# salesforce/ai-economist

Hardware: AMD Instinct MI355X
Metric: agent-steps/sec, gather-trade-build 25x25 4-agent batched envs (higher is better)
Workload: dtype u8/i32 state + f64 coin/utility (f32 observations); 1 GPU; C2 BASELINE configs[1]: gather-trade-build 25x25, 4 agents + planner, Build+CDA+Gather+PeriodicBracketTax, 4096 replicas/GPU, uniform random policy, planner not counted; envs_per_gpu=4096, global_envs=4096, n_agents=4, kernel_specialisation=compile time, parallelism=single GPU

## Files before the change

### ai-economist_amd/csrc/aie_capi.hip

```cpp
#include <hip/hip_runtime.h>

#include <cstdio>
#include <cstdlib>
#include <cstring>
#include <vector>

#include "aie_kernels.hip"
#include "aie_kernels_ose.hip"
#include "aie_kernels_saez.hip"
#include "aie_kernels_covid.hip"
#include "aie_jit.h"

struct aie_env {
  aie_params P{};
  aie_params* d_params;
  aie_tensor_table tt;
  uint8_t* arena;
  bool owns_arena;
  size_t vmm_total, vmm_piece;
  int device;
  size_t lds;
  int spec;
  int spec_match;
  hipModule_t jit_mod;
  hipFunction_t jit_step, jit_reset;
  std::shared_ptr<aie_jit::Job> jit_job;
  int pinned_generic;
  float* rew_log;
  int32_t rew_log_slots, rew_log_epoch;
  int cv_taps_f32;
  int log_active;
  char err[512];
};

static thread_local char g_create_err[512] = "";
static inline void aie_jit_poll(aie_env* env);
static bool aie_jit_eligible(const aie_env* env);
static int aie_jit_request(aie_env* env);

#define AIE_DEV_API __attribute__((visibility("default")))

#define AIE_HIP_CHECK(env, expr)                                                          \
  do {                                                                                    \
    hipError_t _e = (expr);                                                               \
    if (_e != hipSuccess) {                                                               \
      snprintf((env)->err, sizeof((env)->err), "%s failed: %s", #expr, hipGetErrorString(_e)); \
      return AIE_E_HIP;                                                                   \
    }                                                                                     \
  } while (0)

static uint8_t* aie_arena_alloc_pieces(int device, size_t bytes, size_t piece_mb, size_t* vmm_total, size_t* vmm_piece);
static uint8_t* aie_arena_alloc(int device, size_t bytes, size_t* vmm_total, size_t* vmm_piece) {
  const char* e_min = getenv("AIE_ARENA_VMM_MIN_MB");
  const char* e_piece = getenv("AIE_ARENA_PIECE_MB");
  const size_t min_mb = e_min ? (size_t)atol(e_min) : 1024;
  return aie_arena_alloc_pieces(device, bytes, bytes >= (min_mb << 20) ? (e_piece ? (size_t)atol(e_piece) : 64) : 0, vmm_total, vmm_piece);
}
static uint8_t* aie_arena_alloc_pieces(int device, size_t bytes, size_t piece_mb, size_t* vmm_total, size_t* vmm_piece) {
  *vmm_total = *vmm_piece = 0;
  void* p = nullptr;
  if (piece_mb > 0) {
    hipMemAllocationProp prop = {};
    prop.type = hipMemAllocationTypePinned;
    prop.location.type = hipMemLocationTypeDevice;
    prop.location.id = device;
    size_t gran = 0;
    if (hipMemGetAllocationGranularity(&gran, &prop, hipMemAllocationGranularityMinimum) == hipSuccess && gran > 0) {
      if (gran < ((size_t)2 << 20)) gran = (size_t)2 << 20;
      size_t piece = (piece_mb << 20) / gran * gran;
      if (piece < gran) piece = gran;
      const size_t total = (bytes + piece - 1) / piece * piece;
      hipDeviceptr_t va = nullptr;
      if (hipMemAddressReserve(&va, total, gran, nullptr, 0) == hipSuccess) {
// ... 236 lines not shown
  int64_t count = 1, span = es;
  for (int i = 0; i < d->ndim; ++i) {
    count *= d->shape[i];
    span += (d->shape[i] - 1) * d->stride[i];
  }
  if (bytes != count * es) {
    snprintf(env->err, sizeof(env->err), "'%s': expected %lld bytes, got %lld", name, (long long)(count * es),
             (long long)bytes);
    return AIE_E_INVALID;
  }
  AIE_HIP_CHECK(env, hipSetDevice(env->device));
  std::vector<uint8_t> tmp((size_t)span);
  uint8_t* dev = env->arena + d->arena_offset;
  AIE_HIP_CHECK(env, hipDeviceSynchronize());
  AIE_HIP_CHECK(env, hipMemcpy(tmp.data(), dev, (size_t)span, hipMemcpyDeviceToHost));
  int64_t idx[6] = {0, 0, 0, 0, 0, 0};
  uint8_t* h = static_cast<uint8_t*>(host);
  for (int64_t k = 0; k < count; ++k) {
    int64_t off = 0;
    for (int i = 0; i < d->ndim; ++i) off += idx[i] * d->stride[i];
    if (upload) memcpy(tmp.data() + off, h + k * es, (size_t)es);
    else memcpy(h + k * es, tmp.data() + off, (size_t)es);
    for (int i = d->ndim - 1; i >= 0; --i) {
      if (++idx[i] < d->shape[i]) break;
      idx[i] = 0;
    }
  }
  if (upload) AIE_HIP_CHECK(env, hipMemcpy(dev, tmp.data(), (size_t)span, hipMemcpyHostToDevice));
  return AIE_OK;
}

int aie_upload(aie_env* env, const char* name, const void* host, int64_t bytes) {
  const int rc = copy_tensor(env, name, const_cast<void*>(host), bytes, true);
  if (rc == AIE_OK && (strcmp(name, "cells") == 0 || strcmp(name, "cell_flags") == 0))
    return aie_rebuild_src_lists(env);
  if (rc == AIE_OK && env->P.c.scenario == AIE_SCN_COVID && strcmp(name, "model_unemp_conv_filters") == 0) {
    const double* taps = static_cast<const double*>(host);
    env->cv_taps_f32 = 1;
    for (int64_t q = 0; q < bytes / 8; ++q)
      if ((double)(float)taps[q] != taps[q]) env->cv_taps_f32 = 0;
  }
  if (rc == AIE_OK && env->P.c.scenario == AIE_SCN_COVID &&
      (strcmp(name, "model_stringency_level_history_0") == 0 || strcmp(name, "model_unemp_conv_filters") == 0)) {
    hipLaunchKernelGGL(aie_covid_prepare_kernel, dim3(1), dim3(AIE_NT), 0, 0, env->d_params, env->arena);
    AIE_HIP_CHECK(env, hipGetLastError());
    AIE_HIP_CHECK(env, hipDeviceSynchronize());
  }
  return rc;
}
int aie_download(aie_env* env, const char* name, void* host, int64_t bytes) {
  return copy_tensor(env, name, host, bytes, false);
}

int aie_set_layout(aie_env* env, const uint8_t* stone_src, const uint8_t* wood_src, const uint8_t* water) {
  if (!env) return AIE_E_INVALID;
  if (env->P.c.scenario != AIE_SCN_GTB) return AIE_OK;
  if (!stone_src || !wood_src) return AIE_E_INVALID;
  const aie_params& P = env->P;
  const int shared = P.c.shared_layout ? 1 : 0;
  const int64_t cnt = (shared ? 1 : (int64_t)P.E) * P.HW;
  std::vector<uint8_t> fl((size_t)cnt);
  for (int64_t q = 0; q < cnt; ++q)
    fl[(size_t)q] = (uint8_t)(((water && water[q]) ? AIE_CELL_WATER : 0u) | (stone_src[q] ? AIE_CELL_STONE_SRC : 0u) |
                              (wood_src[q] ? AIE_CELL_WOOD_SRC : 0u));
  AIE_HIP_CHECK(env, hipSetDevice(env->device));
  uint8_t* dfl = nullptr;
// ... 259 lines not shown
           else { \
             hipLaunchKernelGGL((aie_covid_step_kernel<FN, false>), g, b, 0, st, env->d_params, env->arena, d_actions_a, d_actions_p, next); \
             if (env->cv_taps_f32) hipLaunchKernelGGL((aie_covid_window_kernel<FN, float>), gw, bw, lw, st, env->d_params, env->arena); \
             else hipLaunchKernelGGL((aie_covid_window_kernel<FN, double>), gw, bw, lw, st, env->d_params, env->arena); \
           } \
           break
    switch (env->P.cv_F) {
      AIE_CV_LAUNCH(1); AIE_CV_LAUNCH(2); AIE_CV_LAUNCH(3); AIE_CV_LAUNCH(4);
      AIE_CV_LAUNCH(5); AIE_CV_LAUNCH(6); AIE_CV_LAUNCH(7); AIE_CV_LAUNCH(8);
      default: return AIE_E_UNSUPPORTED;
    }
#undef AIE_CV_LAUNCH
  } else if (env->P.c.scenario == AIE_SCN_ONE_STEP_ECONOMY && env->spec == AIE_KERNEL_INSTANCE_JIT) {
    const aie_params* dp = env->d_params;
    uint8_t* ar = env->arena;
    NextActions nx = next;
    void* args[] = {&dp, &ar, &d_actions_a, &d_actions_p, &nx};
    AIE_HIP_CHECK(env, hipModuleLaunchKernel(env->jit_step, (unsigned)env->P.E, 1, 1, OSE_NT, 1, 1, (unsigned)env->lds,
                                             static_cast<hipStream_t>(stream), args, nullptr));
  } else if (env->P.c.scenario == AIE_SCN_ONE_STEP_ECONOMY && env->spec >= 0) {
    const dim3 g((unsigned)env->P.E), b(OSE_NT);
    hipStream_t st = static_cast<hipStream_t>(stream);
#define AIE_SPEC_LAUNCH_OSE(K) \
  case K: hipLaunchKernelGGL(aie_ose_step_kernel_spec<K>, g, b, env->lds, st, env->d_params, env->arena, d_actions_a, d_actions_p, next); break;
    switch (env->spec) {
      AIE_SPEC_LIST_OSE(AIE_SPEC_LAUNCH_OSE)
      default: return AIE_E_INVALID;
    }
#undef AIE_SPEC_LAUNCH_OSE
  } else if (env->P.c.scenario == AIE_SCN_ONE_STEP_ECONOMY)
    hipLaunchKernelGGL(aie_ose_step_kernel, dim3((unsigned)env->P.E), dim3(OSE_NT), env->lds,
                       static_cast<hipStream_t>(stream), env->d_params, env->arena, d_actions_a, d_actions_p, next);
#ifdef AIE_DEV
  else if (env->spec >= 0 && !(env->P.dev_skip_mask & (1 << 20)) && (env->P.dev_trace != nullptr || env->P.dev_skip_mask != 0)) {
    const dim3 g((unsigned)env->P.E), b(2 * AIE_NT);
    hipStream_t st = static_cast<hipStream_t>(stream);
#define AIE_SPEC_LAUNCH_TR(K) \
  case K: hipLaunchKernelGGL(aie_step_kernel_spec_trace<K>, g, b, env->lds, st, env->d_params, env->arena, d_actions_a, d_actions_p, next); break;
    switch (env->spec) {
      AIE_SPEC_LIST_GTB(AIE_SPEC_LAUNCH_TR)
      default: return AIE_E_INVALID;
    }
#undef AIE_SPEC_LAUNCH_TR
  }
#endif
  else if (env->P.saez_stride || env->P.M > AIE_NT || env->P.regen_general || env->P.dev_skip_mask != 0 ||
           env->P.dev_trace != nullptr || env->P.n_host_a || env->P.n_host_p)
    hipLaunchKernelGGL(aie_step_kernel_log, dim3((unsigned)env->P.E), dim3(2 * AIE_NT), env->lds,
                       static_cast<hipStream_t>(stream), env->d_params, env->arena, d_actions_a, d_actions_p, next);
  else if (env->spec == AIE_KERNEL_INSTANCE_JIT) {
    const aie_params* dp = env->d_params;
    uint8_t* ar = env->arena;
    NextActions nx = next;
    void* args[] = {&dp, &ar, &d_actions_a, &d_actions_p, &nx};
    AIE_HIP_CHECK(env, hipModuleLaunchKernel(env->jit_step, (unsigned)env->P.E, 1, 1, 2 * AIE_NT, 1, 1, (unsigned)env->lds,
                                             static_cast<hipStream_t>(stream), args, nullptr));
  } else if (env->spec >= 0) {
    const dim3 g((unsigned)env->P.E), b(2 * AIE_NT);
    hipStream_t st = static_cast<hipStream_t>(stream);
#define AIE_SPEC_LAUNCH(K) \
  case K: hipLaunchKernelGGL(aie_step_kernel_spec<K>, g, b, env->lds, st, env->d_params, env->arena, d_actions_a, d_actions_p, next); break;
    switch (env->spec) {
      AIE_SPEC_LIST_GTB(AIE_SPEC_LAUNCH)
      default: return AIE_E_INVALID;
    }
#undef AIE_SPEC_LAUNCH
  } else if (aie_workgroups_per_cu(env->lds) <= 12)
// ... 478 lines not shown
AIE_DEV_API int aie_dev_lds_bytes(aie_env* env, int64_t* out) {
  if (!env || !out) return AIE_E_INVALID;
  out[0] = (int64_t)env->lds;
  out[5] = aie_workgroups_per_cu(env->lds);
  out[1] = env->P.o_mt;
  out[2] = env->P.HW;
  out[3] = env->P.c.scenario == AIE_SCN_ONE_STEP_ECONOMY || env->P.c.scenario == AIE_SCN_COVID ? 0 : (int64_t)aie::fscr_doubles(env->P) * 8;
  out[4] = env->P.c.scenario == AIE_SCN_ONE_STEP_ECONOMY || env->P.c.scenario == AIE_SCN_COVID ? 0 : (int64_t)aie::stage_bytes(env->P);
  return AIE_OK;
}

static int aie_dev_push_params(aie_env* env) {
  AIE_HIP_CHECK(env, hipSetDevice(env->device));
  AIE_HIP_CHECK(env, hipDeviceSynchronize());
  AIE_HIP_CHECK(env, hipMemcpy(env->d_params, &env->P, sizeof(aie_params), hipMemcpyHostToDevice));
  return AIE_OK;
}

AIE_DEV_API int aie_dev_set_trace(aie_env* env, void* d_buf) {
  if (!env) return AIE_E_INVALID;
  env->P.dev_trace = static_cast<uint64_t*>(d_buf);
  return aie_dev_push_params(env);
}

AIE_DEV_API int aie_dev_set_lds_pad(aie_env* env, int bytes) {
  if (!env || bytes < 0) return AIE_E_INVALID;
  env->lds += (size_t)bytes;
  return AIE_OK;
}

AIE_DEV_API int aie_dev_set_draw_window(aie_env* env, int words) {
  if (!env || words < 0) return AIE_E_INVALID;
  env->P.dev_draw_window = words;
  env->P.dev_skip_mask = words ? (env->P.dev_skip_mask | (1 << 20)) : (env->P.dev_skip_mask & ~(1 << 20));
  return aie_dev_push_params(env);
}

AIE_DEV_API int aie_dev_set_skip_mask(aie_env* env, int mask) {
  if (!env) return AIE_E_INVALID;
  env->P.dev_skip_mask = mask;
  return aie_dev_push_params(env);
}
#endif

}
```

### ai-economist_amd/csrc/aie_kernels.hip

```cpp
#pragma once
#include <hip/hip_runtime.h>
#include <stdint.h>

#include "aie_layout.h"
#include "aie_glibc_math.h"

#pragma clang fp contract(off)

#ifdef AIE_JIT
#include "aie_jit_image.h"
#else
#include "aie_spec_generated.h"
#endif
template <int SPEC>
__device__ __forceinline__ const aie_params& aie_spec_params(const aie_params* run_time) {
  if constexpr (SPEC < 0) return *run_time;
  else return *reinterpret_cast<const aie_params*>(aie_spec_image<SPEC>::bytes);
}

#define AIE_NT 64
#define AIE_DIRTY_CAP 64

namespace aie {

// ... 667 lines not shown
  const int o = AIE_CELL_OWNER(w);
  if (!(o < 0 || o == agent)) return false;
  const int occ = c.locmap[cell];
  return occ == 0 || occ == agent + 1;
}

__device__ __forceinline__ void log_event(const Ctx& c, int type, int a1, int a2, int a3, int a4, int a5,
                                          int a6, int a7, int a8, double f) {
  if (c.tid != 0) return;
  const int k = c.srcn[2];
  if (k >= c.R.ev_cap) return;
  int32_t* row = c.ev + 4 + k * AIE_EV_WORDS;
  row[0] = type; row[1] = a1; row[2] = a2; row[3] = a3; row[4] = a4;
  row[5] = a5; row[6] = a6; row[7] = a7; row[8] = a8; row[9] = 0;
  *reinterpret_cast<double*>(row + 10) = f;
  c.srcn[2] = k + 1;
}

__device__ __forceinline__ bool agent_can_build(const Ctx& c, int i) {
  const int n = c.P.n;
  const int32_t* inv = R_I32(c, o_inv_res);
  if (inv[n + i] < 1 || inv[i] < 1) return false;
  const uint32_t w = R_CELLS(c)[R_I32(c, o_loc_r)[i] * c.P.W + R_I32(c, o_loc_c)[i]];
  return (w & 0xffffu) == 0 && ((w >> 16) & 0xffu) == 0xffu && (w >> 24) == 0;
}

struct Agents {
  int lr, lc;
  int inv0, inv1;
  int esc0, esc1;
  int no0, no1;
  uint32_t act;
  double coin, esc_coin, labor;
};
#define AIE_ACT_BUILD(a) ((a) & 1u)
#define AIE_ACT_GATHER(a) (((a) >> 1) & 7u)
#define AIE_ACT_BUY(a, r) (((a) >> (4 + 14 * (r))) & 0x7fu)
#define AIE_ACT_SELL(a, r) (((a) >> (11 + 14 * (r))) & 0x7fu)

__device__ __forceinline__ void agents_load(const Ctx& c, Agents& A) {
  const int n = c.P.n, i = c.tid < n ? c.tid : 0;
  A.lr = R_I32(c, o_loc_r)[i];
  A.lc = R_I32(c, o_loc_c)[i];
  A.inv0 = R_I32(c, o_inv_res)[i];
  A.inv1 = R_I32(c, o_inv_res)[n + i];
  A.esc0 = R_I32(c, o_esc_res)[i];
  A.esc1 = R_I32(c, o_esc_res)[n + i];
  A.no0 = c.P.has_cda ? R_I32(c, o_cda_n_orders)[i] : 0;
  A.no1 = c.P.has_cda ? R_I32(c, o_cda_n_orders)[n + i] : 0;
  A.coin = R_F64(c, o_inv_coin)[i];
  A.esc_coin = R_F64(c, o_esc_coin)[i];
  A.labor = R_F64(c, o_labor)[i];
}
__device__ __forceinline__ void agents_store(const Ctx& c, const Agents& A) {
  const int n = c.P.n, i = c.tid;
  if (i < n) {
    R_I32(c, o_loc_r)[i] = A.lr;
    R_I32(c, o_loc_c)[i] = A.lc;
    R_I32(c, o_inv_res)[i] = A.inv0;
    R_I32(c, o_inv_res)[n + i] = A.inv1;
    R_I32(c, o_esc_res)[i] = A.esc0;
    R_I32(c, o_esc_res)[n + i] = A.esc1;
    if (c.P.has_cda) {
      R_I32(c, o_cda_n_orders)[i] = A.no0;
      R_I32(c, o_cda_n_orders)[n + i] = A.no1;
    }
    R_F64(c, o_inv_coin)[i] = A.coin;
// ... 326 lines not shown
__device__ __forceinline__ void hist_add(uint8_t* hist, int idx, int lane) {
  if (lane == 0) atomicAdd(reinterpret_cast<uint32_t*>(hist + (idx & ~3)), 1u << (8 * (idx & 3)));
}
__device__ __forceinline__ void hist_sub_lane(uint8_t* hist, int idx) {
  atomicSub(reinterpret_cast<uint32_t*>(hist + (idx & ~3)), 1u << (8 * (idx & 3)));
}

__device__ __forceinline__ void cda_component_step(const Ctx& c, Agents& A) {
  const int n = c.P.n, M = c.P.M, P = c.P.P, lane = c.tid;
  const int maxo = c.P.c.cda_max_num_orders, dur = c.R.c.cda_order_duration;
  uint8_t* bid_hist = R_U8(c, o_cda_bid_hist);
  uint8_t* ask_hist = R_U8(c, o_cda_ask_hist);
  int nb[2] = {uni(R_I32(c, o_cda_n_bids)[0]), uni(R_I32(c, o_cda_n_bids)[1])};
  int na[2] = {uni(R_I32(c, o_cda_n_asks)[0]), uni(R_I32(c, o_cda_n_asks)[1])};
  const int nb0[2] = {nb[0], nb[1]}, na0[2] = {na[0], na[1]};

#pragma unroll
  for (int r = 0; r < AIE_N_RES; ++r) {
    int32_t* bids = R_I32(c, o_cda_bids) + r * M;
    int32_t* asks = R_I32(c, o_cda_asks) + r * M;
    const uint32_t buy = AIE_ACT_BUY(A.act, r), sell = AIE_ACT_SELL(A.act, r);
    const uint64_t mb = __ballot(lane < n && buy > 0), ms = __ballot(lane < n && sell > 0);
    uint64_t mm = mb | ms;
    while (mm) {
      const int i = __ffsll((unsigned long long)mm) - 1;
      mm &= mm - 1;
      const int no = bcast(r ? A.no1 : A.no0, i);
      if ((mb >> i) & 1ull) {
        const int price = (int)bcast(buy, i) - 1;
        if (no < maxo && !(bcast(A.coin, i) < (double)price)) {
          bids[nb[r]] = AIE_ORD_PACK(i, price, 0);
          nb[r] += 1;
          hist_add(bid_hist, (r * n + i) * P + price, lane);
          if (lane == i) {
            if (r) A.no1 += 1; else A.no0 += 1;
            const double tr = A.coin < (double)price ? A.coin : (double)price;
            A.coin -= tr;
            A.esc_coin += tr;
            A.labor += c.R.c.cda_order_labor;
          }
        }
      }
      if ((ms >> i) & 1ull) {
        const int price = (int)bcast(sell, i) - 1;
        const int no2 = bcast(r ? A.no1 : A.no0, i);
        if (no2 < maxo && bcast(r ? A.inv1 : A.inv0, i) > 0) {
          asks[na[r]] = AIE_ORD_PACK(i, price, 0);
          na[r] += 1;
          hist_add(ask_hist, (r * n + i) * P + price, lane);
          if (lane == i) {
            if (r) { A.no1 += 1; A.inv1 -= 1; A.esc1 += 1; }
            else { A.no0 += 1; A.inv0 -= 1; A.esc0 += 1; }
            A.labor += c.R.c.cda_order_labor;
          }
        }
      }
    }
  }

#pragma unroll
  for (int r = 0; r < AIE_N_RES; ++r) {
    int32_t* bids = R_I32(c, o_cda_bids) + r * M;
    int32_t* asks = R_I32(c, o_cda_asks) + r * M;
    if (nb[r] == nb0[r] && na[r] == na0[r]) continue;
    uint64_t possible = (n >= 64) ? ~0ull : ((1ull << n) - 1ull);
    if (!c.full || M <= AIE_NT) {
      int32_t bv = lane < nb[r] ? bids[lane] : 0;
      int32_t av = lane < na[r] ? asks[lane] : 0;
      for (int q = nb0[r]; q < nb[r]; ++q) {
        const int32_t x = bcast(bv, q);
        const int pb = __popcll(__ballot(lane < q && !order_before<true>(x, bv)));
        const int32_t up = (int32_t)__builtin_amdgcn_update_dpp(0, bv, 0x138 , 0xf, 0xf, false);
        bv = (lane > pb && lane <= q) ? up : bv;
        bv = (lane == pb) ? x : bv;
      }
      for (int q = na0[r]; q < na[r]; ++q) {
        const int32_t x = bcast(av, q);
        const int pa = __popcll(__ballot(lane < q && !order_before<false>(x, av)));
        const int32_t up = (int32_t)__builtin_amdgcn_update_dpp(0, av, 0x138 , 0xf, 0xf, false);
        av = (lane > pa && lane <= q) ? up : av;
        av = (lane == pa) ? x : av;
      }
      uint64_t alive_b = nb[r] >= 64 ? ~0ull : ((1ull << nb[r]) - 1ull);
      uint64_t alive_a = na[r] >= 64 ? ~0ull : ((1ull << na[r]) - 1ull);
      if (nb[r] == 0 || na[r] == 0) possible = 0;
      const int my_buyer = AIE_ORD_AGENT(bv), my_seller = AIE_ORD_AGENT(av);
      int ntrades = 0, trade = 0;
      while (possible) {
        const uint64_t bh = __ballot((possible >> my_buyer) & 1ull) & alive_b;
        if (!bh) break;
        const int ib = __ffsll((unsigned long long)bh) - 1;
        const int32_t bid = bcast(bv, ib);
        const int buyer = AIE_ORD_AGENT(bid), bprice = AIE_ORD_PRICE(bid);
        const uint64_t ah = __ballot(my_seller != buyer) & alive_a;
        int ia = -1;
        int32_t ask = 0;
        if (ah) { ia = __ffsll((unsigned long long)ah) - 1; ask = bcast(av, ia); }
        if (ia < 0 || bprice < AIE_ORD_PRICE(ask)) {
          possible &= ~(1ull << buyer);
          continue;
        }
        alive_b &= ~(1ull << ib);
        alive_a &= ~(1ull << ia);
        const int seller = AIE_ORD_AGENT(ask), aprice = AIE_ORD_PRICE(ask);
        const bool at_ask = AIE_ORD_LIFE(bid) <= AIE_ORD_LIFE(ask);
        const int price = at_ask ? aprice : bprice;
        if (lane == ntrades) trade = buyer | (seller << 6) | (bprice << 12) | (aprice << 20) | ((int)at_ask << 28);
        ntrades += 1;
        if (c.ev) log_event(c, AIE_EV_TRADE, r, seller, buyer, aprice, bprice, price, AIE_ORD_LIFE(ask), AIE_ORD_LIFE(bid), 0.0);
        if (lane == seller) {
          if (r) { A.no1 -= 1; A.esc1 -= 1; } else { A.no0 -= 1; A.esc0 -= 1; }
          A.coin += (double)price;
        }
        if (lane == buyer) {
          if (r) { A.no1 -= 1; A.inv1 += 1; } else { A.no0 -= 1; A.inv0 += 1; }
          A.esc_coin -= (double)bprice;
          A.coin += (double)(bprice - price);
        }
      }
      if (lane < ntrades) {
        const int buyer = trade & 63, seller = (trade >> 6) & 63, bprice = (trade >> 12) & 255, aprice = (trade >> 20) & 255;
        const int price = ((trade >> 28) & 1) ? aprice : bprice;
        const int bi = (r * n + buyer) * P + bprice, ai = (r * n + seller) * P + aprice;
        atomicSub(reinterpret_cast<uint32_t*>(bid_hist + (bi & ~3)), 1u << (8 * (bi & 3)));
        atomicSub(reinterpret_cast<uint32_t*>(ask_hist + (ai & ~3)), 1u << (8 * (ai & 3)));
        unsafeAtomicAdd(R_F64(c, o_cda_price_history) + (r * n + seller) * P + price, 1.0);
        if (C_MET(c)) {
          int32_t* tm = reinterpret_cast<int32_t*>(C_MET(c) + c.P.mo_cda);
          int32_t* sell = tm + ((0 * AIE_N_RES + r) * n + seller) * 2;
          int32_t* buy = tm + ((1 * AIE_N_RES + r) * n + buyer) * 2;
          atomicAdd(sell, 1); atomicAdd(sell + 1, price);
          atomicAdd(buy, 1); atomicAdd(buy + 1, price);
        }
      }
      AIE_WSYNC();
      if ((alive_b >> lane) & 1ull) bids[__popcll(alive_b & ((1ull << lane) - 1ull))] = bv;
      if ((alive_a >> lane) & 1ull) asks[__popcll(alive_a & ((1ull << lane) - 1ull))] = av;
      nb[r] = __popcll(alive_b);
      na[r] = __popcll(alive_a);
      AIE_WSYNC();
      continue;
    }
    for (int q = nb0[r]; q < nb[r]; ++q) book_insert<true>(bids, q, lane);
    for (int q = na0[r]; q < na[r]; ++q) book_insert<false>(asks, q, lane);
    if (nb[r] == 0 || na[r] == 0) continue;
    while (possible) {
      const uint64_t poss = possible;
      const int ib = book_find_first(bids, nb[r], lane, [poss](int32_t o) { return ((poss >> AIE_ORD_AGENT(o)) & 1ull) != 0; });
      if (ib < 0) break;
      const int32_t bid = uni(bids[ib]);
      const int buyer = AIE_ORD_AGENT(bid), bprice = AIE_ORD_PRICE(bid);
      const int ia = book_find_first(asks, na[r], lane, [buyer](int32_t o) { return AIE_ORD_AGENT(o) != buyer; });
      int32_t ask = 0;
      if (ia >= 0) ask = uni(asks[ia]);
      if (ia < 0 || bprice < AIE_ORD_PRICE(ask)) {
        possible &= ~(1ull << buyer);
        continue;
      }
      book_remove(bids, nb[r], ib, lane);
      nb[r] -= 1;
      book_remove(asks, na[r], ia, lane);
      na[r] -= 1;
      const int seller = AIE_ORD_AGENT(ask), aprice = AIE_ORD_PRICE(ask);
      const int price = (AIE_ORD_LIFE(bid) <= AIE_ORD_LIFE(ask)) ? aprice : bprice;
      bid_hist[(r * n + buyer) * P + bprice] -= 1;
      ask_hist[(r * n + seller) * P + aprice] -= 1;
      R_F64(c, o_cda_price_history)[(r * n + seller) * P + price] += 1.0;
      if (lane == 0 && C_MET(c)) {
        int32_t* tm = reinterpret_cast<int32_t*>(C_MET(c) + c.P.mo_cda);
        int32_t* sell = tm + ((0 * AIE_N_RES + r) * n + seller) * 2;
        int32_t* buy = tm + ((1 * AIE_N_RES + r) * n + buyer) * 2;
        atomicAdd(sell, 1); atomicAdd(sell + 1, price);
        atomicAdd(buy, 1); atomicAdd(buy + 1, price);
      }
      if (c.ev) log_event(c, AIE_EV_TRADE, r, seller, buyer, aprice, bprice, price, AIE_ORD_LIFE(ask), AIE_ORD_LIFE(bid), 0.0);
      if (lane == seller) {
        if (r) { A.no1 -= 1; A.esc1 -= 1; } else { A.no0 -= 1; A.esc0 -= 1; }
        A.coin += (double)price;
      }
      if (lane == buyer) {
        if (r) { A.no1 -= 1; A.inv1 += 1; } else { A.no0 -= 1; A.inv0 += 1; }
        A.esc_coin -= (double)bprice;
        A.coin += (double)(bprice - price);
      }
    }
  }

  if (!c.full || M <= AIE_NT) {
    int32_t ob[2][2];
#pragma unroll
    for (int r = 0; r < AIE_N_RES; ++r) {
      ob[r][0] = lane < nb[r] ? (R_I32(c, o_cda_bids) + r * M)[lane] : 0;
      ob[r][1] = lane < na[r] ? (R_I32(c, o_cda_asks) + r * M)[lane] : 0;
    }
    AIE_WSYNC();
#pragma unroll
    for (int r = 0; r < AIE_N_RES; ++r) {
#pragma unroll
      for (int side = 0; side < 2; ++side) {
        int32_t* v = (side == 0 ? R_I32(c, o_cda_bids) : R_I32(c, o_cda_asks)) + r * M;
        const int len = side == 0 ? nb[r] : na[r];
        const int32_t o = ob[r][side];
        const bool valid = lane < len;
        const int life = AIE_ORD_LIFE(o) + 1;
        const bool keep = valid && life <= dur;
        const uint64_t km = __ballot(keep);
        uint64_t em = __ballot(valid && !keep);
        if (keep) v[__popcll(km & lanemask_lt(lane))] = AIE_ORD_PACK(AIE_ORD_AGENT(o), AIE_ORD_PRICE(o), life);
        if (valid && !keep) hist_sub_lane(side == 0 ? bid_hist : ask_hist, (r * n + AIE_ORD_AGENT(o)) * P + AIE_ORD_PRICE(o));
        while (em) {
          const int q = __ffsll((unsigned long long)em) - 1;
          em &= em - 1;
          const int32_t eo = bcast(o, q);
          const int ag = AIE_ORD_AGENT(eo), pr = AIE_ORD_PRICE(eo);
          if (lane == ag) {
            if (side == 0) {
              const double tr = A.esc_coin < (double)pr ? A.esc_coin : (double)pr;
              A.esc_coin -= tr;
              A.coin += tr;
              if (r) A.no1 -= 1; else A.no0 -= 1;
            } else {
              if (r) { A.esc1 -= 1; A.inv1 += 1; A.no1 -= 1; }
              else { A.esc0 -= 1; A.inv0 += 1; A.no0 -= 1; }
            }
          }
        }
        if (side == 0) nb[r] = __popcll(km); else na[r] = __popcll(km);
      }
    }
  } else {
#pragma unroll
  for (int r = 0; r < AIE_N_RES; ++r) {
#pragma unroll
    for (int side = 0; side < 2; ++side) {
      int32_t* v = (side == 0 ? R_I32(c, o_cda_bids) : R_I32(c, o_cda_asks)) + r * M;
      const int len = side == 0 ? nb[r] : na[r];
      int kept = 0;
      for (int base = 0; base < len; base += AIE_NT) {
        const int idx = base + lane;
        const bool valid = idx < len;
        const int32_t o = valid ? v[idx] : 0;
        const int life = AIE_ORD_LIFE(o) + 1;
        const bool keep = valid && life <= dur;
        const uint64_t km = __ballot(keep);
        uint64_t em = __ballot(valid && !keep);
        if (keep) v[kept + __popcll(km & lanemask_lt(lane))] = AIE_ORD_PACK(AIE_ORD_AGENT(o), AIE_ORD_PRICE(o), life);
        kept += __popcll(km);
        while (em) {
          const int q = __ffsll((unsigned long long)em) - 1;
          em &= em - 1;
          const int32_t eo = bcast(o, q);
          const int ag = AIE_ORD_AGENT(eo), pr = AIE_ORD_PRICE(eo);
          if (side == 0) {
            bid_hist[(r * n + ag) * P + pr] -= 1;
            if (lane == ag) {
              const double tr = A.esc_coin < (double)pr ? A.esc_coin : (double)pr;
              A.esc_coin -= tr;
              A.coin += tr;
              if (r) A.no1 -= 1; else A.no0 -= 1;
            }
          } else {
            ask_hist[(r * n + ag) * P + pr] -= 1;
            if (lane == ag) {
              if (r) { A.esc1 -= 1; A.inv1 += 1; A.no1 -= 1; }
              else { A.esc0 -= 1; A.inv0 += 1; A.no0 -= 1; }
            }
          }
        }
      }
      if (side == 0) nb[r] = kept; else na[r] = kept;
    }
  }
  }
  R_I32(c, o_cda_n_bids)[0] = nb[0];
  R_I32(c, o_cda_n_bids)[1] = nb[1];
  R_I32(c, o_cda_n_asks)[0] = na[0];
  R_I32(c, o_cda_n_asks)[1] = na[1];
}

#pragma clang fp contract(off)
__device__ __forceinline__ double tax_curr_rate_max(const Ctx& c) {
  return aie_annealed_tax_limit(*R_I32(c, o_tax_last_completions), c.R.c.tax_annealing_warmup,
                                c.R.c.tax_annealing_slope, c.R.c.tax_rate_max);
}
__device__ __forceinline__ uint8_t* saez_block(const Ctx& c) {
// ... 105 lines not shown
    R_F64(c, o_tax_last_coin)[i] = A.coin + A.esc_coin;
  }
  if (c.saez) {
    uint8_t* blk = saez_block(c);
    int32_t* hdr = reinterpret_cast<int32_t*>(blk);
    double* buf = reinterpret_cast<double*>(blk + AIE_SAEZ_OFF_BUF);
    int len = uni(hdr[0]);
    if (i < n) {
      buf[2 * (len + i)] = R_F64(c, o_tax_last_income)[i];
      buf[2 * (len + i) + 1] = R_F64(c, o_tax_last_marginal_rate)[i];
    }
    len += n;
    const int size = c.R.c.saez_buffer_size;
    if (len > size) {
      const int shift = 2 * (len - size);
      __builtin_amdgcn_s_waitcnt(0);
      for (int base = 0; base < 2 * size; base += AIE_NT) {
        const int q = base + i;
        double v = 0;
        if (q < 2 * size) v = buf[q + shift];
        __builtin_amdgcn_s_waitcnt(0);
        if (q < 2 * size) buf[q] = v;
      }
      len = size;
    }
    if (i == 0) {
      hdr[0] = len;
      hdr[2] += n;
    }
  }
}
__device__ __forceinline__ void tax_component_step(const Ctx& c, MTL& ml, Agents& A) {
  int pos = uni(*R_I32(c, o_tax_cycle_pos));
  if (pos == 1 && c.saez) {
    uint8_t* blk = saez_block(c);
    if (uni(reinterpret_cast<const int32_t*>(blk)[1])) {
      if (c.tid < c.P.NB) R_F64(c, o_tax_saez_rates)[c.tid] = reinterpret_cast<const double*>(blk + AIE_SAEZ_OFF_NEXT)[c.tid];
    } else {
      const double lo = c.R.c.tax_rate_min;
      const double hi = c.P.c.tax_annealing ? tax_curr_rate_max(c) : c.R.c.tax_rate_max;
      for (int b = 0; b < c.P.NB; ++b) {
        const double r = lo + (hi - lo) * rng_double(ml, c.tid);
        if (c.tid == b) R_F64(c, o_tax_saez_rates)[b] = r;
      }
    }
    AIE_WSYNC();
    if (c.tid < c.P.NB) R_F64(c, o_tax_saez_obs_rates)[c.tid] = tax_rate(c, c.tid);
    AIE_WSYNC();
  }
  if (pos == 1 && c.P.c.tax_model == AIE_TAX_MODEL_WRAPPER && !c.P.c.tax_disable) {
    if (c.tid < c.P.NB) {
      const int a = c.act_p[c.tid];
      if (a > 0 && a <= c.P.c.tax_n_disc_rates) R_I32(c, o_tax_rate_idx)[c.tid] = a - 1;
    }
    AIE_WSYNC();
  }
  if (pos >= c.R.c.tax_period) {
    tax_enact(c, A);
    pos = 0;
  }
  *R_I32(c, o_tax_cycle_pos) = pos + 1;
}

__device__ __forceinline__ void wealth_component_step(const Ctx& c, Agents& A) {
  const int n = c.P.n;
  const double v = A.coin + A.esc_coin;
// ... 620 lines not shown
    }
  }
  if (P.has_tax && !(skip & 256)) {
    const int pos = *R_I32(c, o_tax_cycle_pos);
    const float is_tax_day = pos >= c.R.c.tax_period ? 1.0f : 0.0f;
    const float is_first_day = pos == 1 ? 1.0f : 0.0f;
    const float tax_phase = (float)((double)pos / (double)c.R.c.tax_period);
    const int fragA = NB + n + 4;
    for (int q = tid; q < (n + 1) * fragA; q += AIE_NT) {
      const int i = udiv(q, fragA, P.mg_taxA);
      const int j = q - i * fragA;
      const bool planner = i == n;
      if (j == NB + 2 + n) {
        if (planner) s_pflat[P.fp_tax + NB + 2 + n] = tax_phase;
        continue;
      }
      if (planner && j == NB + 3 + n) continue;
      float v;
      if (j < NB) v = (float)tax_rate_obs(c, j);
      else if (j == NB) v = is_first_day;
      else if (j == NB + 1) v = is_tax_day;
      else if (j < NB + 2 + n) v = (float)scr_sorted_inc(c)[j - NB - 2];
      else v = tax_phase;
      if (planner) s_pflat[P.fp_tax + j] = v;
      else AF(i * P.FA + P.fa_tax + j, v);
    }
  }

  AIE_WSYNC();

  if (!(skip & 1024)) {
    stream_out(s_pag, reinterpret_cast<float*>(arena + c.R.a_obs_p_agents) + (int64_t)c.e * n * P.FPA, n * P.FPA, tid);
    stream_out(s_pflat, reinterpret_cast<float*>(arena + c.R.a_obs_p_flat) + (int64_t)c.e * P.FP, P.FP, tid);
  }
}


__device__ __forceinline__ void write_action_masks(const Ctx& c, uint8_t* __restrict__ arena, bool all = true) {
  const aie_params& P = c.P;
  const int n = P.n, tid = c.tid, Pp = P.P;
  const int skip = c.skipm;
  if (skip & 512) return;
  if (!P.o_mask_bits) all = true;
  if (tid < n) {
    const int i = tid;
    const double coin = R_F64(c, o_inv_coin)[i];
    const int inv0 = R_I32(c, o_inv_res)[i], inv1 = R_I32(c, o_inv_res)[n + i];
    const int lr = R_I32(c, o_loc_r)[i], lc = R_I32(c, o_loc_c)[i];
    uint32_t mf = 0;
    if (P.has_build) mf |= agent_can_build(c, i) ? 1u : 0u;
    if (P.has_gather) {
      mf |= can_agent_occupy(c, lr, lc - 1, i) ? 2u : 0u;
      mf |= can_agent_occupy(c, lr, lc + 1, i) ? 4u : 0u;
      mf |= can_agent_occupy(c, lr - 1, lc, i) ? 8u : 0u;
      mf |= can_agent_occupy(c, lr + 1, lc, i) ? 16u : 0u;
    }
    if (P.has_cda) {
      int kmax = coin >= (double)(Pp - 1) ? Pp - 1 : (int)coin;
#pragma unroll
      for (int r = 0; r < 2; ++r) {
        const bool quota = R_I32(c, o_cda_n_orders)[r * n + i] < P.c.cda_max_num_orders;
        if (quota && (r ? inv1 : inv0) > 0) mf |= 32u << r;
        if (quota) mf |= (uint32_t)(kmax + 1) << (8 + 8 * r);
      }
    }
    const bool changed = all || (int32_t)mf != R_I32(c, o_mask_bits)[i];
// ... 150 lines not shown
  const int skip = (LOG || TRACE) ? R.dev_skip_mask : 0;
#else
  const int skip = 0;
#endif
  static_assert(NW == 2, "a replica is a workgroup of two wavefronts");
  const int e_blk = replica_of_block((int)blockIdx.x, next.E);
  if (next.e_hi > 0 && (e_blk < next.e_lo || e_blk >= next.e_hi)) return;
  if (LOG && next.mask && !next.mask[e_blk]) return;
  const bool FAST = rng_fast(P);
  const int tid0 = (int)(threadIdx.x & (AIE_NT - 1));
  uint8_t* grec = arena + (int64_t)e_blk * P.rec_bytes;
  uint32_t* gkey = reinterpret_cast<uint32_t*>(grec + P.o_mt);
  const Ctx c = make_ctx(P, R, lds, e_blk, tid0, arena, LOG, skip,
                         SPEC >= 0);
  const bool SHL = shared_src_list(P);
  uint32_t* const draw_w = reinterpret_cast<uint32_t*>(c.stage);
  int draw_cap = stage_window_words(P);
  if (LOG && R.dev_draw_window > 0 && R.dev_draw_window < draw_cap) draw_cap = R.dev_draw_window;
#ifdef AIE_W0_TAIL_PRIO
  const int w0_tail_prio = AIE_W0_TAIL_PRIO;
#else
  const int w0_tail_prio = P.n >= 8 ? 2 : 0;
#endif
  const bool REW_ON_W1 = FAST && P.n < 8;
  const int ph = LOG ? next.phase : 0;
  const bool HEAD = ph == 0 || (ph & 1), TAIL = ph == 0 || (ph & 2), OBSERVE = ph != 0 && (ph & 4) && !(ph & 2);
  const bool REBASE = OBSERVE && (ph & 8);
  const bool RETAX = OBSERVE && (ph & 16);
  const bool REGEN = TAIL || (ph & 64), EMIT = TAIL || (ph & 128), CLOSE = TAIL || (ph & 256);
  const bool CLOSE_ONLY = CLOSE && !EMIT;
  const int c_lo = ph ? next.comp_lo : 0, c_hi = ph ? next.comp_hi : P.c.n_components;
  if (wid == 0) {
    Agents A;
    int act_err = 0;
    if (!(skip & (1 << 18))) act_err = decode_actions(c, A, act_a, act_p, arena);
    else A.act = 0;
    if (TRACE && R.dev_trace && c.tid == 0) R.dev_trace[12 * blockIdx.x] = wall_clock64();
    if (TRACE && R.dev_trace && c.tid == 0) R.dev_trace[12 * blockIdx.x + 9] = wall_clock64();
    MT none;
    load_record(c, arena, none, 0, NW, -1);
    __syncthreads();
    if (TRACE && R.dev_trace && c.tid == 0) R.dev_trace[12 * blockIdx.x + 8] = wall_clock64();
    MTL ml{draw_w, 0, 0u, -AIE_MT_N, 0, 0u, 0u, 0, 0, 0, FAST ? reinterpret_cast<uint32_t*>(c.rec + P.o_mt) : gkey, draw_cap, FAST};
    ml.pos = ml.base = uni(*R_I32(c, o_mt_pos));
    ml.avail = ml.cap < AIE_MT_N - ml.pos ? ml.cap : AIE_MT_N - ml.pos;
    if (FAST) {
      const int covered = 128 * ((ml.cap + 127) >> 7) - (ml.pos & 1);
      if (ml.avail > covered) ml.avail = covered;
    }
    agents_load(c, A);
    if (act_err && c.tid == 0) *R_I32(c, o_error_flags) |= act_err;
    bool cda_in_range = ph == 0;
    if (ph != 0)
      for (int k = c_lo; k < c_hi; ++k) cda_in_range |= P.c.components[k] == AIE_COMP_CDA;
    if (P.has_cda && !(skip & 1) && cda_in_range) cda_decay_price_history(c);
    __syncthreads();
    if (c.tid == 0 && HEAD) *R_I32(c, o_timestep) += 1;
    if (c.ev && c.tid == 0) c.srcn[2] = 0;
    __builtin_amdgcn_s_setprio(3);
    if (TRACE && R.dev_trace && c.tid == 0) R.dev_trace[12 * blockIdx.x + 1] = wall_clock64();
    if (!(skip & 1)) {
      for (int k = c_lo; k < c_hi; ++k) {
        switch (P.c.components[k]) {
          case AIE_COMP_BUILD: if (!(skip & 2048)) build_component_step(c, ml, A); break;
          case AIE_COMP_CDA: if (!(skip & 4096)) cda_component_step(c, A); break;
          case AIE_COMP_GATHER: if (!(skip & 8192)) gather_component_step(c, ml, A); break;
          case AIE_COMP_TAX: if (!(skip & 16384)) tax_component_step(c, ml, A); break;
          case AIE_COMP_WEALTH_REDISTRIBUTION: wealth_component_step(c, A); break;
          default: break;
        }
        if (TRACE && R.dev_trace && c.tid == 0 && k < 4) R.dev_trace[12 * blockIdx.x + 2 + k] = wall_clock64();
      }
    }
    __builtin_amdgcn_s_setprio(0);
    agents_store(c, A);
    if (c.ev && c.tid == 0) c.ev[0] = c.srcn[2];
    if (c.tid == 0) {
      *R_I32(c, o_mt_pos) = ml.pos;
      c.dirty[0] = ml.dn;
      c.dirty[1] = (int32_t)ml.mv0;
      c.dirty[2] = (int32_t)ml.mv1;
      c.dirty[3] = ml.tw;
    }
    if (TRACE && R.dev_trace && c.tid == 0) R.dev_trace[12 * blockIdx.x + 5] = wall_clock64();
    __syncthreads();
    if (w0_tail_prio) __builtin_amdgcn_s_setprio(2);
    if (RETAX && P.has_tax) {
      if (c.tid < P.n) R_F64(c, o_tax_last_coin)[c.tid] = R_F64(c, o_inv_coin)[c.tid] + R_F64(c, o_esc_coin)[c.tid];
      AIE_WSYNC();
    }
    if (!(skip & 8) && (EMIT || OBSERVE)) write_flat_observations(c, arena);
    if (TRACE && R.dev_trace && c.tid == 0) R.dev_trace[12 * blockIdx.x + 10] = wall_clock64();
    if (!REW_ON_W1 && (EMIT || CLOSE)) step_rewards_and_done(c, arena, next, skip, EMIT, CLOSE);
    if (REBASE) {
      AIE_WSYNC();
      current_metrics(c);
      AIE_WSYNC();
      if (c.tid <= P.n) R_F64(c, o_util)[c.tid] = scr_part(c)[c.tid];
      AIE_WSYNC();
    }
    if (w0_tail_prio) __builtin_amdgcn_s_setprio(0);
    __syncthreads();
    if (!(skip & 32)) store_record_step(c, arena, 0, NW);
    if (TRACE && R.dev_trace && c.tid == 0) R.dev_trace[12 * blockIdx.x + 7] = wall_clock64();
  } else {
    MT m;
    mt_init(m, P);
    const int gpos = *reinterpret_cast<const int32_t*>(grec + P.o_mt_pos);
    load_record(c, arena, m, 1, NW, -1);
    if (skip & (1 << 16)) {}
    else if (FAST) draw_window_publish_fast(draw_w, draw_cap, (uint32_t)uni((int)gkey[0]), (uint32_t)uni((int)gkey[1]), (uint32_t)uni((int)gkey[2]), uni(gpos), c.tid);
    else draw_window_publish_from_hbm(draw_w, draw_cap, gkey, uni(gpos), c.tid);

    if (SPEC >= 0 && const_tables_in_lds(P)) {
      if (P.has_tax && P.c.tax_model == AIE_TAX_MODEL_WRAPPER)
        for (int q = c.tid; q < P.c.tax_n_disc_rates; q += AIE_NT) const_cast<double*>(c.rtab)[q] = R.c.tax_disc_rates[q];
      for (int q = c.tid; q < P.MA; q += AIE_NT) const_cast<uint32_t*>(c.mtab)[q] = P.mask_test[q];
    }
    __syncthreads();
    if (!(skip & (1 << 17))) rebuild_locmap(c);
    __syncthreads();
    SrcList src;
    src.S = 0;
#pragma unroll
// ... 1686 lines not shown
```

Baseline: 699.5 million agent-steps/s.

## Update flat observations incrementally using dirty bits for CDA histograms and tax

Adds per-step dirty tracking for CDA bid/ask histogram columns and tax-state changes, then takes an incremental path that rewrites only changed histogram entries plus the always-changing per-agent, time and tax fields. When the state is not dirty it skips the full flat-observation rewrite. An obs_valid flag in each record gates the fast path, and host uploads into the record region clear that flag so the next step falls back to a full write. The added bookkeeping and branching cost registers in the step kernel. Correctness depends on every histogram mutation site setting its dirty bit.

Measured after the change: 731.5 million agent-steps/s (median of 6 runs). 1.05x the previous value.

```diff
diff --git a/ai-economist_amd/csrc/aie_capi.hip b/ai-economist_amd/csrc/aie_capi.hip
--- a/ai-economist_amd/csrc/aie_capi.hip
+++ b/ai-economist_amd/csrc/aie_capi.hip
@@ -39,6 +39,7 @@
 static int aie_jit_request(aie_env* env);
 
 #define AIE_DEV_API __attribute__((visibility("default")))
+#define AIE_DEV_GENERIC_KERNEL (1 << 30)
 
 #define AIE_HIP_CHECK(env, expr)                                                          \
   do {                                                                                    \
@@ -341,6 +342,13 @@
 
 int aie_upload(aie_env* env, const char* name, const void* host, int64_t bytes) {
   const int rc = copy_tensor(env, name, const_cast<void*>(host), bytes, true);
+  if (rc == AIE_OK && env->P.o_obs_valid && strcmp(name, "obs_valid") != 0) {
+    const aie_tensor_desc* d = find_tensor(env, name);
+    const int64_t r0 = env->P.a_records, r1 = r0 + (int64_t)env->P.E * env->P.rec_bytes;
+    if (d->arena_offset >= r0 && d->arena_offset < r1)
+      AIE_HIP_CHECK(env, hipMemset2DAsync(env->arena + r0 + env->P.o_obs_valid, (size_t)env->P.rec_bytes, 0, 4,
+                                          (size_t)env->P.E, nullptr));
+  }
   if (rc == AIE_OK && (strcmp(name, "cells") == 0 || strcmp(name, "cell_flags") == 0))
     return aie_rebuild_src_lists(env);
   if (rc == AIE_OK && env->P.c.scenario == AIE_SCN_COVID && strcmp(name, "model_unemp_conv_filters") == 0) {
@@ -666,7 +674,7 @@
     hipLaunchKernelGGL(aie_ose_step_kernel, dim3((unsigned)env->P.E), dim3(OSE_NT), env->lds,
                        static_cast<hipStream_t>(stream), env->d_params, env->arena, d_actions_a, d_actions_p, next);
 #ifdef AIE_DEV
-  else if (env->spec >= 0 && !(env->P.dev_skip_mask & (1 << 20)) && (env->P.dev_trace != nullptr || env->P.dev_skip_mask != 0)) {
+  else if (env->spec >= 0 && !(env->P.dev_skip_mask & AIE_DEV_GENERIC_KERNEL) && (env->P.dev_trace != nullptr || env->P.dev_skip_mask != 0)) {
     const dim3 g((unsigned)env->P.E), b(2 * AIE_NT);
     hipStream_t st = static_cast<hipStream_t>(stream);
 #define AIE_SPEC_LAUNCH_TR(K) \
@@ -1211,7 +1219,7 @@
 AIE_DEV_API int aie_dev_set_draw_window(aie_env* env, int words) {
   if (!env || words < 0) return AIE_E_INVALID;
   env->P.dev_draw_window = words;
-  env->P.dev_skip_mask = words ? (env->P.dev_skip_mask | (1 << 20)) : (env->P.dev_skip_mask & ~(1 << 20));
+  env->P.dev_skip_mask = words ? (env->P.dev_skip_mask | AIE_DEV_GENERIC_KERNEL) : (env->P.dev_skip_mask & ~AIE_DEV_GENERIC_KERNEL);
   return aie_dev_push_params(env);
 }
 
diff --git a/ai-economist_amd/csrc/aie_kernels.hip b/ai-economist_amd/csrc/aie_kernels.hip
--- a/ai-economist_amd/csrc/aie_kernels.hip
+++ b/ai-economist_amd/csrc/aie_kernels.hip
@@ -723,7 +723,15 @@
   int no0, no1;
   uint32_t act;
   double coin, esc_coin, labor;
+  uint64_t hist_dirty;
+  bool tax_dirty;
 };
+__device__ __forceinline__ uint64_t hist_bit(const aie_params& P, int r, int side, int price) {
+  return 4 * P.P <= 64 ? 1ull << ((2 * r + side) * P.P + price) : 1ull << (2 * r + side);
+}
+__device__ __forceinline__ bool hist_col_dirty(const aie_params& P, uint64_t dirty, int r, int side, int price) {
+  return ((dirty >> (4 * P.P <= 64 ? (2 * r + side) * P.P + price : 2 * r + side)) & 1ull) != 0;
+}
 #define AIE_ACT_BUILD(a) ((a) & 1u)
 #define AIE_ACT_GATHER(a) (((a) >> 1) & 7u)
 #define AIE_ACT_BUY(a, r) (((a) >> (4 + 14 * (r))) & 0x7fu)
@@ -1116,6 +1124,7 @@
           bids[nb[r]] = AIE_ORD_PACK(i, price, 0);
           nb[r] += 1;
           hist_add(bid_hist, (r * n + i) * P + price, lane);
+          A.hist_dirty |= hist_bit(c.P, r, 1, price);
           if (lane == i) {
             if (r) A.no1 += 1; else A.no0 += 1;
             const double tr = A.coin < (double)price ? A.coin : (double)price;
@@ -1132,6 +1141,7 @@
           asks[na[r]] = AIE_ORD_PACK(i, price, 0);
           na[r] += 1;
           hist_add(ask_hist, (r * n + i) * P + price, lane);
+          A.hist_dirty |= hist_bit(c.P, r, 0, price);
           if (lane == i) {
             if (r) { A.no1 += 1; A.inv1 -= 1; A.esc1 += 1; }
             else { A.no0 += 1; A.inv0 -= 1; A.esc0 += 1; }
@@ -1190,6 +1200,7 @@
         const bool at_ask = AIE_ORD_LIFE(bid) <= AIE_ORD_LIFE(ask);
         const int price = at_ask ? aprice : bprice;
         if (lane == ntrades) trade = buyer | (seller << 6) | (bprice << 12) | (aprice << 20) | ((int)at_ask << 28);
+        A.hist_dirty |= hist_bit(c.P, r, 1, bprice) | hist_bit(c.P, r, 0, aprice);
         ntrades += 1;
         if (c.ev) log_event(c, AIE_EV_TRADE, r, seller, buyer, aprice, bprice, price, AIE_ORD_LIFE(ask), AIE_ORD_LIFE(bid), 0.0);
         if (lane == seller) {
@@ -1249,6 +1260,7 @@
       const int price = (AIE_ORD_LIFE(bid) <= AIE_ORD_LIFE(ask)) ? aprice : bprice;
       bid_hist[(r * n + buyer) * P + bprice] -= 1;
       ask_hist[(r * n + seller) * P + aprice] -= 1;
+      A.hist_dirty |= hist_bit(c.P, r, 1, bprice) | hist_bit(c.P, r, 0, aprice);
       R_F64(c, o_cda_price_history)[(r * n + seller) * P + price] += 1.0;
       if (lane == 0 && C_MET(c)) {
         int32_t* tm = reinterpret_cast<int32_t*>(C_MET(c) + c.P.mo_cda);
@@ -1297,6 +1309,7 @@
           em &= em - 1;
           const int32_t eo = bcast(o, q);
           const int ag = AIE_ORD_AGENT(eo), pr = AIE_ORD_PRICE(eo);
+          A.hist_dirty |= hist_bit(c.P, r, side == 0 ? 1 : 0, pr);
           if (lane == ag) {
             if (side == 0) {
               const double tr = A.esc_coin < (double)pr ? A.esc_coin : (double)pr;
@@ -1335,6 +1348,7 @@
           em &= em - 1;
           const int32_t eo = bcast(o, q);
           const int ag = AIE_ORD_AGENT(eo), pr = AIE_ORD_PRICE(eo);
+          A.hist_dirty |= hist_bit(c.P, r, side == 0 ? 1 : 0, pr);
           if (side == 0) {
             bid_hist[(r * n + ag) * P + pr] -= 1;
             if (lane == ag) {
@@ -1506,6 +1520,8 @@
 }
 __device__ __forceinline__ void tax_component_step(const Ctx& c, MTL& ml, Agents& A) {
   int pos = uni(*R_I32(c, o_tax_cycle_pos));
+  A.tax_dirty |= (pos == 1 && (c.saez || (c.P.c.tax_model == AIE_TAX_MODEL_WRAPPER && !c.P.c.tax_disable))) ||
+                 pos >= c.R.c.tax_period;
   if (pos == 1 && c.saez) {
     uint8_t* blk = saez_block(c);
     if (uni(reinterpret_cast<const int32_t*>(blk)[1])) {
@@ -2192,6 +2208,113 @@
   if (!(skip & 1024)) {
     stream_out(s_pag, reinterpret_cast<float*>(arena + c.R.a_obs_p_agents) + (int64_t)c.e * n * P.FPA, n * P.FPA, tid);
     stream_out(s_pflat, reinterpret_cast<float*>(arena + c.R.a_obs_p_flat) + (int64_t)c.e * P.FP, P.FP, tid);
+  }
+}
+
+__device__ __forceinline__ void update_flat_observations(const Ctx& c, uint8_t* __restrict__ arena, uint64_t hist_dirty) {
+  const aie_params& P = c.P;
+  const int n = P.n, tid = c.tid, Pp = P.P, NB = P.NB;
+  const double isc = P.c.allow_observation_scaling ? 0.01 : 1.0;
+  const BufRsrc aflat = make_rsrc(arena + c.R.a_obs_a_flat + (int64_t)c.e * n * P.FA * 4, (uint32_t)(n * P.FA * 4));
+  auto AF = [&](int idx, float v) { buf_store_f32(aflat, v, 4 * idx, 0); };
+  float* const pflat = reinterpret_cast<float*>(arena + c.R.a_obs_p_flat) + (int64_t)c.e * P.FP;
+  float* const pag = reinterpret_cast<float*>(arena + c.R.a_obs_p_agents) + (int64_t)c.e * n * P.FPA;
+  const int t = *R_I32(c, o_timestep);
+  const float tval = (float)((double)t / (P.c.allow_observation_scaling ? (double)c.R.c.episode_length : 1.0));
+  const int skip = c.skipm;
+  if (P.has_cda && !(skip & 64)) {
+    double* net_ph = scr_net_ph(c);
+    for (int q = tid; q < 2 * Pp; q += AIE_NT) {
+      const int r = q >= Pp ? 1 : 0, k = q - r * Pp;
+      double s = 0;
+      for (int i = 0; i < n; ++i) {
+        const double v = R_F64(c, o_cda_price_history)[(r * n + i) * Pp + k];
+        s = (i == 0) ? v : s + v;
+      }
+      net_ph[q] = s;
+      if (s != 0 && !(skip & 128)) {
+        const float v = (float)(s * isc);
+        pflat[P.fp_cda + 4 * Pp + 2 + q] = v;
+        for (int i = 0; i < n; ++i) AF(i * P.FA + P.fa_cda + 8 * Pp + 2 + q, v);
+      }
+#pragma unroll
+      for (int side = 0; side < 2; ++side) {
+        if (!hist_col_dirty(P, hist_dirty, r, side, k) || (skip & 128)) continue;
+        const uint8_t* h = side ? R_U8(c, o_cda_bid_hist) : R_U8(c, o_cda_ask_hist);
+        int f = 0;
+        for (int i = 0; i < n; ++i) f += h[(r * n + i) * Pp + k];
+        const float full = (float)f;
+        pflat[P.fp_cda + 2 * side * Pp + q] = full;
+        for (int i = 0; i < n; ++i) {
+          const float my = (float)h[(r * n + i) * Pp + k];
+          const int fc = i * P.FA + P.fa_cda;
+          AF(fc + 2 * side * Pp + q, full - my);
+          AF(fc + (4 + 2 * side) * Pp + 2 + q, my);
+        }
+      }
+    }
+  }
+  if (tid < n && !(skip & 64)) {
+    const int i = tid;
+    const int f0 = i * P.FA;
+    const double coin = R_F64(c, o_inv_coin)[i];
+    const int inv0 = R_I32(c, o_inv_res)[i], inv1 = R_I32(c, o_inv_res)[n + i];
+    const int lr = R_I32(c, o_loc_r)[i], lc = R_I32(c, o_loc_c)[i];
+    AF(f0 + P.fa_time, tval);
+    const float w0 = (float)(coin * isc);
+    const float w1 = (float)((double)inv0 * isc);
+    const float w2 = (float)((double)inv1 * isc);
+    const float w3 = (float)((double)lc / (double)P.W);
+    const float w4 = (float)((double)lr / (double)P.H);
+    AF(f0 + P.fa_world + 0, w0); AF(f0 + P.fa_world + 1, w1); AF(f0 + P.fa_world + 2, w2);
+    float* q = pag + i * P.FPA;
+    if (!P.c.full_observability) {
+      AF(f0 + P.fa_world + 3, w3); AF(f0 + P.fa_world + 4, w4);
+      q[P.fpa_world + 0] = w0; q[P.fpa_world + 1] = w1; q[P.fpa_world + 2] = w2;
+      if (P.c.planner_gets_spatial_info) { q[P.fpa_world + 3] = w3; q[P.fpa_world + 4] = w4; }
+    }
+    reinterpret_cast<float*>(arena + c.R.a_obs_a_time)[(int64_t)c.e * n + i] = tval;
+    if (P.has_tax) {
+      const double cmr = tax_marginal_rate(c, (coin + R_F64(c, o_esc_coin)[i]) - R_F64(c, o_tax_last_coin)[i]);
+      AF(f0 + P.fa_tax + NB + 2 + n, (float)cmr);
+      q[P.fpa_tax + 0] = (float)cmr;
+    }
+  }
+  if (tid == 0) {
+    pflat[P.fp_time] = tval;
+    reinterpret_cast<float*>(arena + c.R.a_obs_p_time)[c.e] = tval;
+  }
+  if (P.has_tax && !(skip & 256)) {
+    const int pos = *R_I32(c, o_tax_cycle_pos);
+    const float is_tax_day = pos >= c.R.c.tax_period ? 1.0f : 0.0f;
+    const float is_first_day = pos == 1 ? 1.0f : 0.0f;
+    const float tax_phase = (float)((double)pos / (double)c.R.c.tax_period);
+    for (int i = tid; i <= n; i += AIE_NT) {
+      if (i == n) {
+        pflat[P.fp_tax + NB] = is_first_day;
+        pflat[P.fp_tax + NB + 1] = is_tax_day;
+        pflat[P.fp_tax + NB + 2 + n] = tax_phase;
+      } else {
+        AF(i * P.FA + P.fa_tax + NB, is_first_day);
+        AF(i * P.FA + P.fa_tax + NB + 1, is_tax_day);
+        AF(i * P.FA + P.fa_tax + NB + 3 + n, tax_phase);
+      }
+    }
+  }
+  if (P.has_cda && !(skip & 128)) {
+    AIE_WSYNC();
+    if (tid < 2) {
+      const int r = tid;
+      const double* a = scr_net_ph(c) + r * Pp;
+      double dot = 0;
+      for (int k = 0; k < Pp; ++k) dot += (double)k * a[k];
+      const double tot = np_sum_small(a, Pp);
+      if (tot != 0) {
+        const float mr = (float)(dot / (tot > 0.001 ? tot : 0.001));
+        pflat[P.fp_cda + 4 * Pp + r] = mr;
+        for (int i = 0; i < n; ++i) AF(i * P.FA + P.fa_cda + 4 * Pp + r, mr);
+      }
+    }
   }
 }
 
@@ -2408,6 +2531,8 @@
   const int c_lo = ph ? next.comp_lo : 0, c_hi = ph ? next.comp_hi : P.c.n_components;
   if (wid == 0) {
     Agents A;
+    A.hist_dirty = 0;
+    A.tax_dirty = false;
     int act_err = 0;
     if (!(skip & (1 << 18))) act_err = decode_actions(c, A, act_a, act_p, arena);
     else A.act = 0;
@@ -2425,6 +2550,11 @@
       if (ml.avail > covered) ml.avail = covered;
     }
     agents_load(c, A);
+#ifdef AIE_FLAT_FULL
+    const bool flat_in_place = false;
+#else
+    const bool flat_in_place = ph == 0 && uni(*R_I32(c, o_obs_valid)) != 0 && !(skip & (1 << 20));
+#endif
     if (act_err && c.tid == 0) *R_I32(c, o_error_flags) |= act_err;
     bool cda_in_range = ph == 0;
     if (ph != 0)
@@ -2465,7 +2595,11 @@
       if (c.tid < P.n) R_F64(c, o_tax_last_coin)[c.tid] = R_F64(c, o_inv_coin)[c.tid] + R_F64(c, o_esc_coin)[c.tid];
       AIE_WSYNC();
     }
-    if (!(skip & 8) && (EMIT || OBSERVE)) write_flat_observations(c, arena);
+    if (!(skip & 8) && (EMIT || OBSERVE)) {
+      const bool annealed_first = P.has_tax && P.c.tax_annealing && uni(*R_I32(c, o_timestep)) == 1;
+      if (flat_in_place && !A.tax_dirty && !annealed_first) update_flat_observations(c, arena, A.hist_dirty);
+      else write_flat_observations(c, arena);
+    }
     if (TRACE && R.dev_trace && c.tid == 0) R.dev_trace[12 * blockIdx.x + 10] = wall_clock64();
     if (!REW_ON_W1 && (EMIT || CLOSE)) step_rewards_and_done(c, arena, next, skip, EMIT, CLOSE);
     if (REBASE) {
```
